# brunohs1993/Nanokappa

Measured on AMD Instinct MI355X. Metric: phonon-steps/sec (whole node), higher is better.
Workload: dtype f64

## Files before the change

### nanokappa_amd/csrc/nk_kernels.h

```cpp
#pragma once
#ifndef NK_KERNEL_LINKAGE
#define NK_KERNEL_LINKAGE
#endif
#include "nk_device.h"

#define NK_TILE 64
#ifndef NK_NT
#define NK_NT 0
#endif
#if NK_NT
#define NK_LD(p) __builtin_nontemporal_load(p)
#define NK_ST(p, v) __builtin_nontemporal_store(v, p)
#else
#define NK_LD(p) (*(p))
#define NK_ST(p, v) (*(p) = (v))
#endif
#ifdef NK_STAMPS
#define NK_STAMP(k)                                                                                    \
    do {                                                                                               \
        unsigned long long t_;                                                                         \
        __builtin_amdgcn_sched_barrier(0);                                                             \
        asm volatile("s_memtime %0\n\ts_waitcnt lgkmcnt(0)" : "=s"(t_)::"memory");                     \
        __builtin_amdgcn_sched_barrier(0);                                                             \
        st_acc[k] += t_ - st_last;                                                                     \
        st_last = t_;                                                                                  \
    } while (0)
#else
#define NK_STAMP(k) do { } while (0)
#endif

__device__ __forceinline__ int nk_rank(unsigned long long m) {
    return (int)__builtin_amdgcn_mbcnt_hi((unsigned int)(m >> 32), __builtin_amdgcn_mbcnt_lo((unsigned int)m, 0u));
}

struct NkLds {
    NkSvTab tb;
    NkBins bins;
    const double *planes, *faces;
    const NkFacet *facets;
    const double *resT;
    const int *rf_off;
    const double *rf_cdf, *rf_verts;
    unsigned int *sp_pref, *sp_cnt, *sp_rm;
    double *sp_cv, *sp_pr;
    double *lrec;
    double *carry;
    double *oring;
    unsigned int *oring_w;
    double *colsum;
};

#ifndef NK_LREC_STRIDE
#define NK_LREC_STRIDE 5
#endif
#ifndef NK_OUT_RING
#define NK_OUT_RING 0
#endif
#define NK_ORING (NK_OUT_RING ? 128 : 0)
#define NK_CARRY_DOUBLES(kind) (((kind) == 3 || (kind) == 5) ? 576 : 448)
#ifndef NK_BOX_GENERAL_CAST
#define NK_BOX_GENERAL_CAST 0
#endif
#define NK_COLSUM_DOUBLES 768
__host__ __device__ inline size_t nk_lds_bytes(int S, int R, int F, int NP, int Fc, int geom, int kind, int nrf, int rbfP, int nlrec = 0, int carry = 0) {
    const bool emit = kind == 1 || kind >= 4;
    int Fl = geom == 1 ? F : 0;
    int Pl = Fl ? NP : 0;
    int Fcl = geom == 1 ? Fc : 0;
    size_t nd = (size_t)S + (size_t)((rbfP + 1) & ~1) + 3 * S + ((3 * S) & 1) + 4 * (size_t)S + NK_NREP * S + NK_NREP * 3 * S + 4 * R +
                (size_t)Fl * NK_FACE_DOUBLES + (size_t)Pl * NK_PLANE_DOUBLES + 2 * (size_t)R + 10 * (size_t)nrf +
                (emit ? 2 * (size_t)(NK_WG / 64) * NK_EMIT_CHUNK : 0) + (kind >= 2 ? (size_t)(NK_WG / 64) * ((size_t)nlrec * 2 * NK_LREC_STRIDE + (carry ? NK_CARRY_DOUBLES(kind) : 0) + NK_ORING * ((kind == 3 || kind == 5) ? 6 : 5)) : 0) +
                (kind >= 4 ? NK_COLSUM_DOUBLES : 0) + 4;
    size_t bytes = nd * 8 + (size_t)Fcl * sizeof(NkFacet) +
                   (size_t)(NK_NREP * S + R + 1 + (R + 1) + (emit ? 3 * (NK_WG / 64) * NK_EMIT_CHUNK : 0) + (kind >= 2 ? (NK_WG / 64) * NK_ORING : 0)) * 4 + 32;
    return (bytes + 15) & ~(size_t)15;
}

template <int GEOM, int KIND>
__device__ __forceinline__ void nk_lds_carve(const NkDev &d, unsigned char *smem, NkLds &L) {
    constexpr bool EMIT = KIND == 1 || KIND >= 4;
    const int S = d.S, R = d.R;
    const int Fl = GEOM == 1 ? d.F : 0;
    const int Pl = Fl ? d.NP : 0;
    const int Fcl = GEOM == 1 ? d.Fc : 0;
    const int nrf = (GEOM == 1 && d.res_lds) ? d.res_nf : 0;
    double *p = (double *)smem;
    L.tb.Tsv = p; p += S + ((d.rbf_P + 1) & ~1);
    L.tb.cen = p; p += 3 * S + ((3 * S) & 1);
    p += ((size_t)S & 1);
    L.tb.sv = (const NkSv *)p; p += 4 * S;
    L.bins.E = p; p += NK_NREP * S;
    L.bins.flux = p; p += NK_NREP * 3 * S;
    L.bins.resb = p; p += 4 * R;
    p += ((size_t)(p - (double *)smem) & 1);
    double *faces = p; p += (size_t)Fl * NK_FACE_DOUBLES;
    double *planes = p; p += (size_t)Pl * NK_PLANE_DOUBLES;
    double *resT = p; p += 2 * R;
    double *rf_cdf = p; p += nrf;
    double *rf_verts = p; p += 9 * (size_t)nrf;
    if (EMIT) { L.sp_cv = p; p += (NK_WG / 64) * NK_EMIT_CHUNK; L.sp_pr = p; p += (NK_WG / 64) * NK_EMIT_CHUNK; } else L.sp_cv = L.sp_pr = nullptr;
    p += ((size_t)(p - (double *)smem) & 1);
    if (KIND >= 2) {
        L.lrec = p; p += (NK_WG / 64) * (size_t)d.nlrec * 2 * NK_LREC_STRIDE;
        L.carry = p; p += d.qx ? 0 : (NK_WG / 64) * NK_CARRY_DOUBLES(KIND);
        L.oring = p; p += (NK_WG / 64) * NK_ORING * ((KIND == 3 || KIND == 5) ? 6 : 5);
    } else { L.lrec = nullptr; L.carry = nullptr; L.oring = nullptr; }
    if (KIND >= 4) { L.colsum = p; p += NK_COLSUM_DOUBLES; } else L.colsum = nullptr;
    NkFacet *facets = (NkFacet *)p;
    unsigned int *u = (unsigned int *)(facets + Fcl);
    L.bins.N = u; u += NK_NREP * S;
    L.bins.nleave = u; u += R;
    L.bins.misc = u; u += 1;
    int *rf_off = (int *)u; u += R + 1;
    if (EMIT) {
        L.sp_pref = u; u += (NK_WG / 64) * NK_EMIT_CHUNK;
        L.sp_cnt = u; u += (NK_WG / 64) * NK_EMIT_CHUNK;
        L.sp_rm = u; u += (NK_WG / 64) * NK_EMIT_CHUNK;
    } else { L.sp_pref = L.sp_cnt = L.sp_rm = nullptr; }
    if (KIND >= 2) { L.oring_w = u; u += (NK_WG / 64) * NK_ORING; } else L.oring_w = nullptr;
    L.resT = resT;
    L.rf_off = rf_off; L.rf_cdf = rf_cdf; L.rf_verts = rf_verts;
    if (GEOM == 1) { L.faces = faces; L.planes = planes; L.facets = facets; }
    else { L.faces = d.faces; L.planes = d.planes; L.facets = d.facets; }
}
template <int GEOM, int KIND>
__device__ __forceinline__ void nk_lds_setup(const NkDev &d, unsigned char *smem, NkLds &L) {
    nk_lds_carve<GEOM, KIND>(d, smem, L);
    const int S = d.S, R = d.R;
    const int Fl = GEOM == 1 ? d.F : 0;
    const int Pl = Fl ? d.NP : 0;
    const int Fcl = GEOM == 1 ? d.Fc : 0;
    const int nrf = (GEOM == 1 && d.res_lds) ? d.res_nf : 0;
    double *faces = const_cast<double *>(L.faces), *planes = const_cast<double *>(L.planes);
    NkFacet *facets = const_cast<NkFacet *>(L.facets);
    double *resT = const_cast<double *>(L.resT), *rf_cdf = const_cast<double *>(L.rf_cdf), *rf_verts = const_cast<double *>(L.rf_verts);
    int *rf_off = const_cast<int *>(L.rf_off);
    double *Tsv = const_cast<double *>(L.tb.Tsv), *cen = const_cast<double *>(L.tb.cen);
    NkSv *sv = const_cast<NkSv *>(L.tb.sv);
    const int t = threadIdx.x, nth = blockDim.x;
    const int nT = S + d.rbf_P, a = d.sv_axis, nface = Fl * NK_FACE_DOUBLES, nplane = Pl * NK_PLANE_DOUBLES;
    const int nfw = Fcl * (int)(sizeof(NkFacet) / 4);
    const int jn = t + 1 < S ? t + 1 : t;
    const double l_T = t < nT ? d.T_sv[t] : 0.0;
    const double l_cen = t < 3 * S ? d.centers[t] : 0.0;
    const double l_c = t < S ? d.centers[3 * t + a] : 0.0, l_cn = t < S ? d.centers[3 * jn + a] : 0.0, l_Tn = t < S ? d.T_sv[jn] : 0.0;
    const double l_rT = t < R ? d.res_T[t] : 1.0;
    const double l_face = t < nface ? d.faces[t] : 0.0;
    const double l_plane = t < nplane ? d.planes[t] : 0.0;
    const int l_off = (nrf > 0 && t <= R) ? d.res_face_off[t] : 0;
    const double l_cdf = t < nrf ? d.res_face_cdf[t] : 0.0;
    const double l_vert = t < 9 * nrf ? d.res_face_verts[t] : 0.0;
    const int32_t l_fw = t < nfw ? ((const int32_t *)d.facets)[t] : 0;
    if (t < nT) Tsv[t] = l_T;
    if (t < 3 * S) cen[t] = l_cen;
    if (t < S) {
        NkSv q;
        q.c = l_c; q.T = l_T; q.slope = jn > t ? (l_Tn - l_T) / (l_cn - l_c) : 0.0; q.invT = 1.0 / l_T;
        sv[t] = q;
    }
    if (t < R) { L.bins.nleave[t] = 0u; resT[2 * t] = l_rT; resT[2 * t + 1] = 1.0 / l_rT; }
    if (t < nface) faces[t] = l_face;
    if (t < nplane) planes[t] = l_plane;
    if (nrf > 0 && t <= R) rf_off[t] = l_off;
    if (t < nrf) rf_cdf[t] = l_cdf;
    if (t < 9 * nrf) rf_verts[t] = l_vert;
    if (t < nfw) ((int32_t *)facets)[t] = l_fw;
    for (int i = t; i < NK_NREP * S; i += nth) { L.bins.E[i] = 0.0; L.bins.N[i] = 0u; }
    for (int i = t; i < NK_NREP * 3 * S; i += nth) L.bins.flux[i] = 0.0;
    for (int i = t; i < 4 * R; i += nth) L.bins.resb[i] = 0.0;
    if (t == 0) L.bins.misc[0] = 0u;
    for (int i = t + nth; i < nT; i += nth) Tsv[i] = d.T_sv[i];
    for (int i = t + nth; i < 3 * S; i += nth) cen[i] = d.centers[i];
    for (int i = t + nth; i < S; i += nth) {
        const int j = i + 1 < S ? i + 1 : i;
        const double c = d.centers[3 * i + a], cn = d.centers[3 * j + a], T = d.T_sv[i], Tn = d.T_sv[j];
        NkSv q;
        q.c = c; q.T = T; q.slope = j > i ? (Tn - T) / (cn - c) : 0.0; q.invT = 1.0 / T;
        sv[i] = q;
    }
    for (int i = t + nth; i < R; i += nth) { L.bins.nleave[i] = 0u; const double T = d.res_T[i]; resT[2 * i] = T; resT[2 * i + 1] = 1.0 / T; }
    for (int i = t + nth; i < nface; i += nth) faces[i] = d.faces[i];
    for (int i = t + nth; i < nplane; i += nth) planes[i] = d.planes[i];
    if (nrf > 0) {
        for (int i = t + nth; i <= R; i += nth) rf_off[i] = d.res_face_off[i];
        for (int i = t + nth; i < nrf; i += nth) rf_cdf[i] = d.res_face_cdf[i];
        for (int i = t + nth; i < 9 * nrf; i += nth) rf_verts[i] = d.res_face_verts[i];
    }
    for (int i = t + nth; i < nfw; i += nth) ((int32_t *)facets)[i] = ((const int32_t *)d.facets)[i];
    __syncthreads();
}

__device__ __forceinline__ void nk_lds_flush(const NkDev &d, const NkLds &L, int64_t row) {
    __syncthreads();
    const int S = d.S, R = d.R;
    double *out = d.partials + row * d.NB;
    for (int b = threadIdx.x; b < d.NB; b += blockDim.x) {
        double v = 0.0;
        if (b < S) { for (int r = 0; r < NK_NREP; ++r) v += L.bins.E[r * S + b]; }
        else if (b < 2 * S) { unsigned int c = 0; for (int r = 0; r < NK_NREP; ++r) c += L.bins.N[r * S + (b - S)]; v = (double)c; }
        else if (b < 5 * S) { int k = b - 2 * S; for (int r = 0; r < NK_NREP; ++r) v += L.bins.flux[r * 3 * S + k]; }
        else if (b < 5 * S + R) v = (double)L.bins.nleave[b - 5 * S];
        else if (b < 5 * S + 2 * R) v = L.bins.resb[4 * (b - 5 * S - R)];
        else if (b < 5 * S + 5 * R) { int k = b - 5 * S - 2 * R; v = L.bins.resb[4 * (k / 3) + 1 + (k % 3)]; }
        else v = (double)L.bins.misc[0];
        out[b] = v;
    }
}

struct NkSegModes {
    const NkMode *rec;
    const int32_t *gm;
    int nl;
    int estride, eoff;
    __device__ __forceinline__ int mode(int i) const { return gm ? gm[i] : i; }
    __device__ __forceinline__ int entry_mode(int l) const { return gm ? gm[l] : l * estride + eoff; }
};
struct NkPlainModes { __device__ __forceinline__ int mode(int i) const { return i; } };
__device__ __forceinline__ void nk_mode_home(const NkDev &d, int mode, int &seg, int &idx) {
    const uint32_t slot = (uint32_t)d.m2s[mode], n = (uint32_t)d.nseg;
    const uint32_t q = slot / n;
    idx = (int)q;
    seg = (int)(slot - q * n);
}
__device__ __forceinline__ NkSegModes nk_seg_modes(const NkDev &d, int seg) {
    NkSegModes sm;
    sm.rec = d.part ? d.modetab_p + (int64_t)seg * d.nlmax : d.modetab;
    sm.gm = d.part ? d.s2m + (int64_t)seg * d.nlmax : nullptr;
    sm.nl = d.seg_nl[seg];
    sm.estride = d.nseg; sm.eoff = seg;
    return sm;
}

template <bool RBF = true>
__device__ __forceinline__ double nk_relax(const NkDev &d, const NkLds &L, const NkTauWin &tw, const double4 &ra, const double4 &rb, double x,
                                           double y, double z, double occ, const NkSegModes &sm, int idx) {
    double invT;
    const double T = nk_interp_T<RBF>(d, L.tb, x, y, z, invT);
    const double tau = nk_lifetime(d, tw, rb.y, rb.z, rb.w, T, sm, idx);
    const double n0 = (T > 0.0) ? nk_be(ra.x * d.c_hk, rb.x, invT, d.invT0) : 0.0;
    const double xr = -d.dt * nk_rcp(tau);
    double er;
    if (__builtin_expect(__ballot(tau > 0.0 && !(xr > -0.125)) == 0ull, 1)) er = nk_exp_small(xr);
    else er = nk_exp(xr);
    return (tau > 0.0) ? n0 + (occ - n0) * er : n0;
}

__device__ __forceinline__ void nk_sample_res_face(const int *off, const double *cdf, const double *verts, int r, double uf,
                                                   double us, double ur, double &x0, double &y0, double &z0) {
    const int f0 = off[r], nf = off[r + 1] - f0;
    int a = nk_ss_right(cdf + f0, nf, uf);
    a = a > nf - 1 ? nf - 1 : a;
    const double *fv = verts + 9 * (f0 + a);
    const double sq = sqrt(us);
    const double a0 = 1.0 - sq, a1 = (1.0 - ur) * sq, a2 = ur * sq;
    x0 = a0 * fv[0] + a1 * fv[3] + a2 * fv[6];
    y0 = a0 * fv[1] + a1 * fv[4] + a2 * fv[7];
    z0 = a0 * fv[2] + a1 * fv[5] + a2 * fv[8];
}

#define NK_RAY(GEOM, d, L, skip, x, y, z, vx, vy, vz, tc, fc)                                                        \
    do {                                                                                                              \
        if ((GEOM) == 2 && (d).NG > 0) nk_find_boundary_tree(d, skip, x, y, z, vx, vy, vz, tc, fc);                      \
        else nk_find_boundary((L).planes, (L).faces, (d).NP, (d).tol, x, y, z, vx, vy, vz, tc, fc);                   \
    } while (0)

__device__ __forceinline__ void nk_emit_entry(const NkDev &d, uint32_t step, int64_t rm, int64_t at, double prob, int &c, int &c_mine, double &cv) {
    const double fixed = floor(prob);
    int mask;
    if (d.res_gen == 0) {
        cv = d.rc_p[(int64_t)(step & 1u) * d.rc_len + at] + (prob - fixed);
        mask = cv >= 1.0;
        cv -= (double)mask;
        d.rc_p[(int64_t)((step + 1u) & 1u) * d.rc_len + at] = cv;
    } else {
        double d1;
        nk_uniform2_dev(d.seed, (uint64_t)rm | 0xFFFFFFFF00000000ull, step, NK_TAG_DICE, cv, d1);
        mask = cv <= (prob - fixed);
    }
    c = (int)fixed + mask;
    c_mine = c;
    if (d.nranks > 1) {
        c_mine = 0;
        for (int level = c; level >= 1; --level)
            c_mine += (((uint32_t)rm + (uint32_t)level + step) % (uint32_t)d.nranks) == (uint32_t)d.rank;
    }
}

NK_KERNEL_LINKAGE __global__ __launch_bounds__(NK_WG) void k_emit_one_to_one(NkDev d, uint32_t step) {
    if (d.halt[0]) return;
    int64_t total = 0;
    for (int r = 0; r < d.R; ++r) total += d.nleave_prev[r];
    for (int64_t c = (int64_t)blockIdx.x * NK_WG + threadIdx.x; c < total; c += (int64_t)gridDim.x * NK_WG) {
        int r = 0;
        int64_t i = c;
        while (r < d.R - 1 && i >= d.nleave_prev[r]) { i -= d.nleave_prev[r]; ++r; }
        if (((uint32_t)((uint64_t)i + step) % (uint32_t)d.nranks) != (uint32_t)d.rank) continue;
        const uint64_t pid = ((uint64_t)((step + 1u) & 0xFFFFFFu) << 40) | ((uint64_t)r << 32) | (uint64_t)i;
        double um, u1;
        nk_uniform2_dev(d.seed, pid, step, NK_TAG_DICE, um, u1);
        int m = nk_ss_left(d.res_roulette + (int64_t)r * d.M, d.M, um);
        m = m > d.M - 1 ? d.M - 1 : m;
        if (i >= (1ll << 24)) { atomicOr(d.overflow, 16); continue; }
        int seg, lidx;
        if (d.part) nk_mode_home(d, m, seg, lidx); else seg = m % d.nseg;
        const int at = atomicAdd(d.sp_inbox_n + seg, 1);
        if (at < d.sp_icap) d.sp_inbox[(int64_t)seg * d.sp_icap + at] = ((uint64_t)i << 40) | ((uint64_t)((int64_t)r * d.M + m) << 12);
        else atomicOr(d.overflow, 8);
    }
}

__device__ __forceinline__ void nk_newborn_place(const NkDev &d, double x0, double y0, double z0, double vx, double vy, double vz,
                                                 double dt_in, double tc, double &x, double &y, double &z, double &nts) {
    x = x0 + vx * dt_in; y = y0 + vy * dt_in; z = z0 + vz * dt_in;
    nts = tc / d.dt - dt_in / d.dt;
}

template <int GEOM, bool BOX>
__device__ __forceinline__ int nk_emit_one(const NkDev &d, const NkLds &L, uint32_t step, int seg, int lane, unsigned int *sp_pref,
                                           unsigned int *sp_cnt, unsigned int *sp_rm, double *sp_cv, double *sp_pr, bool ahead, bool to_queue,
                                           int &bound_out
#ifdef NK_STAMPS
                                           , unsigned long long em_t0, unsigned long long em_t1, unsigned long long &em_t2
#endif
) {
    const int plo = d.seg_lo ? d.seg_lo[seg] : 0;
    const int64_t base = (int64_t)seg * d.segcap;
    const int count = d.seg_count[seg];
    const NkSegModes sm = nk_seg_modes(d, seg);
    const int nent = d.res_gen != 2 ? d.R * sm.nl : 0;
    int made = 0;
    int sp_bound = 0;
    for (int e0 = 0; e0 < nent || (d.res_gen == 2 && e0 == 0); e0 += NK_EMIT_CHUNK) {
        int spn = 0;
        if (d.res_gen == 2) {
            spn = d.sp_inbox_n[seg];
            spn = spn < d.sp_icap ? spn : d.sp_icap;
            sp_bound = lane == 0 ? 2 * spn + 64 : 0;
        } else {
            unsigned int run = 0;
#pragma unroll
            for (int k = 0; k < 2; ++k) {
                const int e = e0 + k * 64 + lane;
                int c = 0, cmine = 0;
                double cv = 0.0, prob = 0.0;
                unsigned int rm32 = 0, rl = 0;
                if (e < nent) {
                    const int r = e / sm.nl, l = e - r * sm.nl;
                    rl = ((unsigned int)r << 12) | ((unsigned int)l << 18);
                    const int64_t rm = (int64_t)r * d.M + sm.entry_mode(l);
                    const int64_t at = ((int64_t)seg * d.R + r) * d.nlmax + l;
                    prob = d.ep_p[at];
                    nk_emit_entry(d, step, rm, at, prob, c, cmine, cv);
                    rm32 = (unsigned int)rm;
                    sp_bound += ((int)floor(prob) + 1 + d.nranks - 1) / d.nranks;
                }
                unsigned int v = (unsigned int)cmine;
#pragma unroll
                for (int o = 1; o < 64; o <<= 1) { const unsigned int u = __shfl_up(v, o, 64); if (lane >= o) v += u; }
                sp_cnt[k * 64 + lane] = (unsigned int)c | rl;
                sp_rm[k * 64 + lane] = rm32;
                sp_cv[k * 64 + lane] = cv;
                sp_pr[k * 64 + lane] = prob;
                sp_pref[k * 64 + lane] = v + run - (unsigned int)cmine;
                run += __shfl(v, 63, 64);
            }
            __builtin_amdgcn_fence(__ATOMIC_SEQ_CST, "wavefront");
            spn = (int)run;
        }
#ifdef NK_STAMPS
        if (!em_t2) em_t2 = __builtin_amdgcn_s_memrealtime();
#endif
        for (int spj = 0; spj < spn; spj += NK_TILE) {
            const int j = spj + lane;
            if (j >= spn) continue;
            int64_t rm;
            int level, r, idx;
            double prob = 0.0, cval = 0.0;
            uint64_t o2o = 0;
            if (d.res_gen == 2) {
                const uint64_t recd = d.sp_inbox[(int64_t)seg * d.sp_icap + j];
                rm = (int64_t)((recd >> 12) & 0xFFFFFFFull);
                level = 0;
                o2o = recd >> 40;
                r = (int)((uint32_t)rm / (uint32_t)d.M);
                const int mode = (int)((uint32_t)rm - (uint32_t)r * (uint32_t)d.M);
                idx = d.part ? (int)((uint32_t)d.m2s[mode] / (uint32_t)d.nseg) : mode;
            } else {
                int lo = 0, hi = NK_EMIT_CHUNK;
                while (hi - lo > 1) { const int mid = (lo + hi) >> 1; if ((int)sp_pref[mid] <= j) lo = mid; else hi = mid; }
                const unsigned int cw = sp_cnt[lo];
                const int q = j - (int)sp_pref[lo], c = (int)(cw & 0xFFFu);
                r = (int)((cw >> 12) & 0x3Fu);
                rm = (int64_t)sp_rm[lo];
                idx = d.part ? (int)(cw >> 18) : (int)((uint32_t)rm - (uint32_t)r * (uint32_t)d.M);
                cval = sp_cv[lo];
                prob = sp_pr[lo];
                if (d.nranks == 1) level = c - q;
                else {
                    const uint32_t n = (uint32_t)d.nranks;
                    const uint32_t tq = ((uint32_t)d.rank + n - (((uint32_t)rm + step) % n)) % n;
                    const uint32_t top = (uint32_t)c - (((uint32_t)c + n - tq) % n);
                    level = (int)(top - (uint32_t)q * n);
                }
            }
            const NkMode *rec = sm.rec + idx;
            const double4 ra = *reinterpret_cast<const double4 *>(rec);
            const double E0 = rec->E0;
            const uint64_t pid = level > 0 ? ((uint64_t)((step + 1u) & 0xFFFFFFu) << 40) | ((uint64_t)rm << 12) | (uint64_t)level
                                           : ((uint64_t)((step + 1u) & 0xFFFFFFu) << 40) | ((uint64_t)r << 32) | o2o;
            double uf, us, ur, ut;
            nk_uniform2_dev(d.seed, pid, step, NK_TAG_EMIT, uf, us);
            nk_uniform2_dev(d.seed, pid, step, NK_TAG_EMIT + 1, ur, ut);
            const double iprob = level > 0 ? nk_rcp(prob) : 0.0;
            const double dt_in = (level == 0) ? d.dt * ut
                               : (level == 1) ? d.dt * (1.0 - cval * iprob)
                                              : d.dt * (1.0 - ((double)(level - 1) + ut) * iprob);
            double x0, y0, z0;
            if (GEOM == 1 && d.res_lds) nk_sample_res_face(L.rf_off, L.rf_cdf, L.rf_verts, r, uf, us, ur, x0, y0, z0);
            else nk_sample_res_face(d.res_face_off, d.res_face_cdf, d.res_face_verts, r, uf, us, ur, x0, y0, z0);
            const double omega = ra.x, vx = ra.y, vy = ra.z, vz = ra.w;
            const double occ = nk_be(omega * d.c_hk, E0, L.resT[2 * r + 1], d.invT0);
            if (GEOM == 2 && to_queue) {
                const int o = made + j;
                if (o < d.segcap) {
                    const int64_t i = base + o;
                    const int rf = d.res_facet[r];
                    const NkFacet &fq = d.facets[rf];
                    const int skip = nk_tree_skip(d, rf, fq.cx, fq.cy, fq.cz, fq.nx, fq.ny, fq.nz, x0, y0, z0, vx, vy, vz);
                    d.qx[i] = x0; d.qy[i] = y0; d.qz[i] = z0; d.qocc[i] = occ; d.qnts[i] = dt_in;
                    d.qw0[i] = NK_NEWBORN | ((uint32_t)((skip == rf ? rf : -1) + 1) << d.lb) | (uint32_t)idx;
                    if (d.qpid) d.qpid[i] = pid;
                } else if (!(ahead && d.halt[1])) atomicOr(d.overflow, 1);
                continue;
            }
            double tc = 0.0;
            int facet = -1;
            int skip = NK_TREE_NO_SKIP;
            if (GEOM == 2 && d.NG > 0) {
                const int rf = d.res_facet[r];
                const NkFacet &fq = d.facets[rf];
                skip = nk_tree_skip(d, rf, fq.cx, fq.cy, fq.cz, fq.nx, fq.ny, fq.nz, x0, y0, z0, vx, vy, vz);
            }
            if (!BOX) NK_RAY(GEOM, d, L, skip, x0, y0, z0, vx, vy, vz, tc, facet);
            const int o = count + made + j;
            if (plo + o < d.segcap) {
                const int64_t i = base + plo + o;
                const NkSlot q = nk_slot(d, i);
                double xa, ya, za, na;
                nk_newborn_place(d, x0, y0, z0, vx, vy, vz, dt_in, tc, xa, ya, za, na);
                d.x.p[q.od] = xa; d.y.p[q.od] = ya; d.z.p[q.od] = za;
                d.occ.p[q.od] = occ;
                if (!BOX) d.nts.p[q.od] = na;
                d.w0.p[q.ow] = BOX ? (NK_NEWBORN | (uint32_t)idx) : (NK_NEWBORN | ((uint32_t)(facet + 1) << d.lb) | (uint32_t)idx);
                if (d.pid) d.pid.p[q.od] = pid;
            } else if (!(ahead && d.halt[1])) atomicOr(d.overflow, 1);
        }
        made += spn;
        __builtin_amdgcn_fence(__ATOMIC_SEQ_CST, "wavefront");
    }
#pragma unroll
    for (int o = 32; o > 0; o >>= 1) sp_bound += __shfl_xor(sp_bound, o, 64);
    const int room = d.segcap - plo - count;
    const int put = (GEOM == 2 && to_queue) ? 0 : (made < room ? made : (room > 0 ? room : 0));
    if (lane == 0) {
        if (GEOM == 2 && to_queue) { d.seg_new[seg] = 0; d.seg_evq[seg] = made < d.segcap ? made : d.segcap; }
        else d.seg_new[seg] = put;
        d.seg_bound[seg] = sp_bound;
        if (d.res_gen == 2) d.sp_inbox_n[seg] = 0;
#ifdef NK_STAMPS
        if (d.stamps) { unsigned long long *w = d.stamps + ((int64_t)d.nseg + seg) * 8 + 4; w[0] = em_t0; w[1] = em_t1; w[2] = em_t2; w[3] = __builtin_amdgcn_s_memrealtime(); }
#endif
    }
    bound_out = sp_bound;
    return put;
}

template <int GEOM, bool BOX = false>
__device__ __forceinline__ void nk_emit_segments(const NkDev &d, NkLds L, uint32_t step, int bid, int nblocks, bool ahead
#ifdef NK_STAMPS
                                                 , unsigned long long em_t0, unsigned long long em_t1
#endif
) {
#ifdef NK_STAMPS
    unsigned long long em_t2 = 0;
#endif
    const int tid = threadIdx.x, lane = tid & 63, wave = __builtin_amdgcn_readfirstlane(tid >> 6);
    unsigned int *sp_pref = L.sp_pref + wave * NK_EMIT_CHUNK, *sp_cnt = L.sp_cnt + wave * NK_EMIT_CHUNK,
                 *sp_rm = L.sp_rm + wave * NK_EMIT_CHUNK;
    double *sp_cv = L.sp_cv + wave * NK_EMIT_CHUNK, *sp_pr = L.sp_pr + wave * NK_EMIT_CHUNK;
    const int nwaves = nblocks * (NK_WG / 64);
    const bool to_queue = GEOM == 2 && d.NG > 0 && d.qx != nullptr;
    for (int seg = bid * (NK_WG / 64) + wave; seg < d.nseg; seg += nwaves) {
        int bound_;
#ifdef NK_STAMPS
        (void)nk_emit_one<GEOM, BOX>(d, L, step, seg, lane, sp_pref, sp_cnt, sp_rm, sp_cv, sp_pr, ahead, to_queue, bound_, em_t0, em_t1, em_t2);
#else
        (void)nk_emit_one<GEOM, BOX>(d, L, step, seg, lane, sp_pref, sp_cnt, sp_rm, sp_cv, sp_pr, ahead, to_queue, bound_);
#endif
    }
}

template <int GEOM, bool BOX = false>
__device__ __forceinline__ void nk_emit_body(const NkDev &d, uint32_t step, unsigned char *smem, int bid, int nblocks, bool ahead = false) {
#ifdef NK_STAMPS
    const unsigned long long em_t0 = __builtin_amdgcn_s_memrealtime();
#endif
    if (d.halt[0]) return;
    NkLds L;
    nk_lds_setup<GEOM, 1>(d, smem, L);
#ifdef NK_STAMPS
    nk_emit_segments<GEOM, BOX>(d, L, step, bid, nblocks, ahead, em_t0, __builtin_amdgcn_s_memrealtime());
#else
    nk_emit_segments<GEOM, BOX>(d, L, step, bid, nblocks, ahead);
#endif
}

template <int GEOM, bool BOX = false>
__global__ __launch_bounds__(NK_WG) void k_emit(NkDev d, uint32_t step) {
    extern __shared__ __align__(16) unsigned char smem[];
    nk_emit_body<GEOM, BOX>(d, step, smem, (int)blockIdx.x, (int)gridDim.x);
}

template <bool PID>
struct NkOut {
    double *x, *y, *z, *occ, *nts, *pid;
    unsigned int *w0;
    int on, ob, wout;
    int64_t m0; int ms, mroom;
    __device__ __forceinline__ void place(int64_t first, int sign, int room) { m0 = first; ms = sign; mroom = room; }
    __device__ __forceinline__ void init(const NkLds &L, int wave) {
        double *p = L.oring + wave * NK_ORING * (PID ? 6 : 5);
        x = p; y = p + NK_ORING; z = p + 2 * NK_ORING; occ = p + 3 * NK_ORING; nts = p + 4 * NK_ORING; pid = PID ? p + 5 * NK_ORING : nullptr;
        w0 = L.oring_w + wave * NK_ORING;
        on = ob = wout = 0;
    }
    __device__ __forceinline__ int reserve(int rank, int n) { const int o = wout + rank; wout += n; return o; }
    template <bool BOX>
    static __device__ __forceinline__ void put_slot(const NkDev &d, int64_t i, double px, double py, double pz, double pocc, double pnts,
                                                    uint32_t pw0, unsigned long long ppid) {
        typedef NkBlock<!BOX, PID> B;
        double *q = B::slot(d.x.p, i);
        NK_ST(q, px); NK_ST(q + B::O_Y, py); NK_ST(q + B::O_Z, pz); NK_ST(q + B::O_OCC, pocc);
        if (!BOX) NK_ST(q + B::O_NTS, pnts);
        if (PID) NK_ST(reinterpret_cast<unsigned long long *>(q + B::O_PID), ppid);
        NK_ST(B::word(d.x.p, i), pw0);
    }
    template <bool BOX = false>
    __device__ __forceinline__ void store(const NkDev &d, int64_t base, bool put, int o, double px, double py, double pz, double pocc,
                                          double pnts, uint32_t pw0, unsigned long long ppid) {
        if (put) {
            if (o < mroom) put_slot<BOX>(d, m0 + ms * (int64_t)o, px, py, pz, pocc, pnts, pw0, ppid);
            else atomicOr(d.overflow, 2);
        }
    }
    template <bool BOX = false>
    __device__ __forceinline__ void push(const NkDev &d, int64_t base, int lane, bool put, int rank, int n, double px, double py,
                                         double pz, double pocc, double pnts, uint32_t pw0, unsigned long long ppid) {
        if (!NK_OUT_RING) {
            if (put) {
                const int o = wout + rank;
                if (o < mroom) put_slot<BOX>(d, m0 + ms * (int64_t)o, px, py, pz, pocc, pnts, pw0, ppid);
                else atomicOr(d.overflow, 2);
            }
            wout += n;
            return;
        }
        if (put) {
            const int e = (ob + on + rank) & (NK_ORING - 1);
            x[e] = px; y[e] = py; z[e] = pz; occ[e] = pocc; nts[e] = pnts; w0[e] = pw0;
            if (PID) pid[e] = __longlong_as_double((long long)ppid);
        }
        on += n;
        __builtin_amdgcn_fence(__ATOMIC_SEQ_CST, "wavefront");
        if (on >= NK_TILE) flush(d, base, lane, NK_TILE);
    }
    __device__ __forceinline__ void flush(const NkDev &d, int64_t base, int lane, int n) {
        if (wout + n <= d.segcap) {
            if (lane < n) {
                const int e = (ob + lane) & (NK_ORING - 1);
                const int64_t i = base + wout + lane;
                d.x[i] = x[e]; d.y[i] = y[e]; d.z[i] = z[e]; d.occ[i] = occ[e]; d.nts[i] = nts[e]; d.w0[i] = w0[e];
                if (PID) d.pid[i] = (unsigned long long)__double_as_longlong(pid[e]);
            }
            wout += n;
        } else if (lane == 0) atomicOr(d.overflow, 2);
        ob = (ob + n) & (NK_ORING - 1);
        on -= n;
        __builtin_amdgcn_fence(__ATOMIC_SEQ_CST, "wavefront");
    }
};

typedef double nk_v2d __attribute__((ext_vector_type(2)));
typedef const __attribute__((address_space(3))) nk_v2d *NkLdsRec;
__device__ __forceinline__ NkLdsRec nk_lds_rec(const double2 *q) { return (NkLdsRec)(const void *)q; }

#ifndef NK_SWEEP_OCC
#define NK_SWEEP_OCC 3
#endif
#ifndef NK_PREFETCH2
#define NK_PREFETCH2 0
#endif
#ifndef NK_PARK_TAU
#define NK_PARK_TAU 1
#endif
#ifndef NK_PRIO_ROT
#define NK_PRIO_ROT 0
#endif
#ifndef NK_DEFER_STORE
#define NK_DEFER_STORE 0
#endif
#ifndef NK_SWEEP_OCC_BIG
#define NK_SWEEP_OCC_BIG 2
#endif
#ifndef NK_SWEEP_OCC_SPLIT
#define NK_SWEEP_OCC_SPLIT 4
#endif
#define NK_SWEEP_BOUND(GEOM, ROUGH, RBF, SPLIT) ((SPLIT) ? NK_SWEEP_OCC_SPLIT : (((GEOM) == 2 || (RBF)) ? NK_SWEEP_OCC_BIG : NK_SWEEP_OCC))
template <int GEOM, bool ROUGH, bool RBF, bool PID, bool SPLIT, bool LREC, int FAST = 0, bool BOX = false>
__device__ __forceinline__ void nk_sweep_body(const NkDev &d, NkLds L, uint32_t step, int do_relax, int flags, int wg, int nwg
#ifdef NK_STAMPS
                                              , unsigned long long st_entry_r
#endif
) {
    static_assert(!BOX || (GEOM == 1 && !SPLIT && !NK_PREFETCH2 && !NK_OUT_RING), "the box store goes with the fused sweep over LDS tables");
    const bool do_flux = (flags & 1) != 0;
    const int tid = threadIdx.x, lane = tid & 63, wave = __builtin_amdgcn_readfirstlane(tid >> 6);
    const int rep = lane & (NK_NREP - 1);
    const uint32_t lbmask = (1u << d.lb) - 1u;
    NkBoxWalls bw;
    if (BOX) bw.load(d);
    NkTauWin tw;
    tw.load(d, NK_PARK_TAU != 0);
    double2 *lrec = reinterpret_cast<double2 *>(L.lrec) + wave * d.nlrec * NK_LREC_STRIDE;
    double *const cX = L.carry ? L.carry + wave * NK_CARRY_DOUBLES(PID ? 3 : 2) : nullptr;
    double *const cP = cX + 6 * 64;
    uint32_t *const cW = reinterpret_cast<uint32_t *>(cX + (PID ? 7 : 6) * 64);
    const int nwaves = nwg * (NK_WG / 64);
#if NK_PRIO_ROT
    const int prio_phase = (int)(wg / (nwg > 3 ? (nwg + 3) / 4 : 1));
#endif
    for (int seg = wg * (NK_WG / 64) + wave; seg < d.nseg; seg += nwaves) {
        const int64_t base = (int64_t)seg * d.segcap;
        const int nnew = d.R > 0 ? d.seg_new[seg] : 0;
        const int count = d.seg_count[seg] + nnew;
        if (lane == 0 && nnew > 0) atomicAdd(&L.bins.misc[0], (unsigned int)nnew);
        const NkSegModes sm = nk_seg_modes(d, seg);
        constexpr bool use_lrec = LREC;
        if (use_lrec) {
            for (int r0 = lane; r0 < sm.nl; r0 += 64) {
                const double4 *g = reinterpret_cast<const double4 *>(sm.rec + r0);
                const double4 a = g[0], b = g[1];
                double2 *q = lrec + r0 * NK_LREC_STRIDE;
                q[0] = make_double2(a.x, a.y); q[1] = make_double2(a.z, a.w); q[2] = make_double2(b.x, b.y); q[3] = make_double2(b.z, b.w);
                if (NK_LREC_STRIDE > 4 && (ROUGH || PID)) *reinterpret_cast<int *>(q + 4) = sm.mode(r0);
            }
            __builtin_amdgcn_fence(__ATOMIC_SEQ_CST, "wavefront");
        }
        auto mode_of = [&](int i) -> int {
            if (use_lrec && NK_LREC_STRIDE > 4) return *(const __attribute__((address_space(3))) int *)(const void *)(lrec + i * NK_LREC_STRIDE + 4);
            return sm.mode(i);
        };
        constexpr bool ALT = GEOM == 1 || SPLIT;
        const bool down = ALT && d.down != 0;
        const int lo = (ALT && d.seg_lo) ? d.seg_lo[seg] : 0, hi = lo + count;
        const int blo = lo & ~(NK_TILE - 1), bhi = count > 0 ? ((hi - 1) & ~(NK_TILE - 1)) : blo;
        const int nA = count > 0 ? (bhi - blo) / NK_TILE + 1 : 0;
        const int wlo = (!down && lo > (d.segcap - count) / 2) ? 0 : lo;
        NkOut<PID> O;
        O.init(L, wave);
        O.place(down ? base + hi - 1 : base + wlo, down ? -1 : 1, down ? count : d.segcap - wlo);
        int qn = SPLIT ? d.seg_evq[seg] : 0;
        if (SPLIT && lane == 0 && qn > 0) atomicAdd(&L.bins.misc[0], (unsigned int)qn);
        int cn = 0;
#ifdef NK_STAMPS
        unsigned long long st_acc[8] = {0, 0, 0, 0, 0, 0, 0, 0}, st_last;
        asm volatile("s_memtime %0\n\ts_waitcnt lgkmcnt(0)" : "=s"(st_last)::"memory");
        const unsigned long long st_c0 = st_last, st_r0 = __builtin_amdgcn_s_memrealtime();
#endif
        constexpr bool PF2 = NK_PREFETCH2 || SPLIT;
        constexpr bool DEFER = (NK_DEFER_STORE || PF2) && !NK_OUT_RING;
        struct NkTileBuf { uint32_t w0; double x, y, z, occ, nts; unsigned long long pid; };
        NkTileBuf bA = {0u, 0, 0, 0, 0, 0, 0ull}, bB = bA;
        auto fetch = [&](NkTileBuf &b, int r) {
            int rr = down ? bhi - r : blo + r;
            rr = rr < 0 ? 0 : (rr < d.segcap - NK_TILE ? rr : d.segcap - NK_TILE);
            const int64_t i0 = base + rr;
            if (PF2) {
                typedef NkBlock<!BOX, PID> B;
                const double *px = B::tile(d.x.p, i0, lane), *py = px + B::O_Y, *pz = px + B::O_Z, *po = px + B::O_OCC, *pn = px + B::O_NTS;
                const uint32_t *pw = B::word(d.x.p, i0) + lane;
                asm volatile("global_load_dword %0, %1, off" : "=v"(b.w0) : "v"(pw) : "memory");
                asm volatile("global_load_dwordx2 %0, %1, off" : "=v"(b.x) : "v"(px) : "memory");
                asm volatile("global_load_dwordx2 %0, %1, off" : "=v"(b.y) : "v"(py) : "memory");
                asm volatile("global_load_dwordx2 %0, %1, off" : "=v"(b.z) : "v"(pz) : "memory");
                asm volatile("global_load_dwordx2 %0, %1, off" : "=v"(b.occ) : "v"(po) : "memory");
                asm volatile("global_load_dwordx2 %0, %1, off" : "=v"(b.nts) : "v"(pn) : "memory");
                if (PID) { const double *pp = px + B::O_PID; asm volatile("global_load_dwordx2 %0, %1, off" : "=v"(b.pid) : "v"(pp) : "memory"); }
                return;
            }
            if (rr + lane >= lo && rr + lane < hi && r < nA * NK_TILE) {
                typedef NkBlock<!BOX, PID> B;
                const double *q = B::tile(d.x.p, i0, lane);
                b.w0 = NK_LD(B::word(d.x.p, i0) + lane); b.x = NK_LD(q); b.y = NK_LD(q + B::O_Y); b.z = NK_LD(q + B::O_Z); b.occ = NK_LD(q + B::O_OCC);
                if (!BOX) b.nts = NK_LD(q + B::O_NTS);
                if (PID) b.pid = NK_LD(reinterpret_cast<const unsigned long long *>(q + B::O_PID));
            }
        };
        auto arrived = [&](NkTileBuf &b) {
            if (!PF2) return;
            if (PID) asm volatile("s_waitcnt vmcnt(7)" : "+v"(b.w0), "+v"(b.x), "+v"(b.y), "+v"(b.z), "+v"(b.occ), "+v"(b.nts), "+v"(b.pid) : : "memory");
            else asm volatile("s_waitcnt vmcnt(6)" : "+v"(b.w0), "+v"(b.x), "+v"(b.y), "+v"(b.z), "+v"(b.occ), "+v"(b.nts) : : "memory");
        };
        auto drained = [&](NkTileBuf &b) {
            if (PF2) asm volatile("s_waitcnt vmcnt(0)" : "+v"(b.w0), "+v"(b.x), "+v"(b.y), "+v"(b.z), "+v"(b.occ), "+v"(b.nts), "+v"(b.pid) : : "memory");
        };
        fetch(bA, 0);
        if (PF2) fetch(bB, NK_TILE);
        bool sdone = false, sev = false;
        int so = 0, sq = 0;
        double sx = 0, sy = 0, sz = 0, socc = 0, snts = 0;
        uint32_t sw0 = 0u;
        unsigned long long spid = 0;
        auto turn = [&](NkTileBuf &buf, const int t) __attribute__((always_inline)) {
            const bool flush = t == nA;
            arrived(buf);
#if NK_PRIO_ROT
            if ((t & ((1 << NK_PRIO_ROT) - 1)) == 0) {
                switch (((t >> NK_PRIO_ROT) + prio_phase) & 3) {
                    case 0: __builtin_amdgcn_s_setprio(0); break;
                    case 1: __builtin_amdgcn_s_setprio(1); break;
                    case 2: __builtin_amdgcn_s_setprio(2); break;
                    default: __builtin_amdgcn_s_setprio(3); break;
                }
            }
#endif
            bool act = false;
            double x = 0, y = 0, z = 0, occ = 0, nts = 0, omega = 0, E0 = 0, vx = 0, vy = 0, vz = 0;
            uint32_t w0 = 0u;
            unsigned long long pid = 0;
            if (!flush) {
                const int r = t * NK_TILE;
                { const int rr = down ? bhi - r : blo + r; act = rr + lane >= lo && rr + lane < hi; }
                w0 = buf.w0; x = buf.x; y = buf.y; z = buf.z; occ = buf.occ; nts = buf.nts; pid = buf.pid;
            }
            if (DEFER) {
                asm volatile("" : "+v"(x), "+v"(y), "+v"(z), "+v"(occ), "+v"(nts), "+v"(w0));
                O.template store<BOX>(d, base, sdone, so, sx, sy, sz, socc, snts, sw0, spid);
                sdone = false;
                if (SPLIT && sev) {
                    if (sq < d.segcap) {
                        const int64_t i = base + sq;
                        d.qx[i] = sx; d.qy[i] = sy; d.qz[i] = sz; d.qocc[i] = socc; d.qnts[i] = snts; d.qw0[i] = sw0;
                        if (PID) d.qpid[i] = spid;
                    }
                }
                sev = false;
            }
            if (PF2) fetch(buf, (t + 2) * NK_TILE);
            if (!flush) {
                const int r = t * NK_TILE;
                if (!PF2) fetch(buf, r + NK_TILE);
                const bool newborn = (w0 & NK_NEWBORN) != 0u;
                w0 &= ~NK_NEWBORN;
                const int idx = act ? (int)(w0 & lbmask) : 0;
                double4 ra, rb;
                if (use_lrec) {
                    const NkLdsRec q = nk_lds_rec(lrec + idx * NK_LREC_STRIDE);
                    const nk_v2d q0 = q[0], q1 = q[1], q2 = q[2], q3 = q[3];
                    ra = make_double4(q0.x, q0.y, q1.x, q1.y); rb = make_double4(q2.x, q2.y, q3.x, q3.y);
                }
                else { const double4 *g = reinterpret_cast<const double4 *>(sm.rec + idx); ra = g[0]; rb = g[1]; }
                omega = ra.x; vx = ra.y; vy = ra.z; vz = ra.w; E0 = rb.x;
#ifdef NK_STAMPS
                { const double fence_ = x + omega; asm volatile("" ::"v"(fence_)); }
#endif
                NK_STAMP(0);
                if (act && !newborn) {
                    if (do_relax) occ = nk_relax<RBF>(d, L, tw, ra, rb, x, y, z, occ, sm, idx);
                    x += vx * d.dt; y += vy * d.dt; z += vz * d.dt;
                    if (!BOX) nts -= 1.0;
                }
#ifdef NK_STAMPS
                { const double fence_ = x + occ; asm volatile("" ::"v"(fence_)); }
#endif
                NK_STAMP(1);
            }
            const bool ev = BOX ? (act && (w0 & NK_LOST) == 0u && nk_box_out(bw, x, y, z, vx, vy, vz)) : (act && nts < 0.0);
            const bool done = act && !ev;
            const unsigned long long mD = __ballot(done), mE = __ballot(ev);
            if (done) nk_tally_one(d, L.tb, L.bins, x, y, z, occ, omega, E0, vx, vy, vz, do_flux, rep);
            if (DEFER) {
                so = O.reserve(nk_rank(mD), __popcll(mD));
                sdone = done; sx = x; sy = y; sz = z; socc = occ; snts = nts; sw0 = w0; spid = pid;
            } else O.template push<BOX>(d, base, lane, done, nk_rank(mD), __popcll(mD), x, y, z, occ, nts, w0, pid);
            NK_STAMP(2);
            if (SPLIT) {
                if (DEFER) { sev = ev; sq = qn + nk_rank(mE); }
                else if (ev) {
                    const int o = qn + nk_rank(mE);
                    if (o < d.segcap) {
                        const int64_t i = base + o;
                        d.qx[i] = x; d.qy[i] = y; d.qz[i] = z; d.qocc[i] = occ; d.qnts[i] = nts; d.qw0[i] = w0;
                        if (PID) d.qpid[i] = pid;
                    }
                }
                qn += __popcll(mE);
                return;
            }
            const int pn = __popcll(mE), erank = nk_rank(mE);
// ... 1628 lines not shown
```

Baseline: 53.40 billion.

## Prefetch emit segment data during LDS setup and batch per-lane mode loads

Adds a batched emit path for GEOM==1 with small reservoir counts. The first segment's header, emission probabilities, carry values and mode records are loaded into registers while the LDS setup loads are still in flight, overlapping that global latency with setup. Mode records are then shared across the wave with shuffles instead of per-entry global loads. For BOX geometry a slim setup also skips loading geometry tables into LDS. This costs more registers and adds a code path that only applies when R<=2 and nlmax<=128.

Measured after the change: 51.95 billion. 2.7% lower.

```diff
diff --git a/nanokappa_amd/csrc/nk_kernels.h b/nanokappa_amd/csrc/nk_kernels.h
--- a/nanokappa_amd/csrc/nk_kernels.h
+++ b/nanokappa_amd/csrc/nk_kernels.h
@@ -123,8 +123,8 @@
     if (GEOM == 1) { L.faces = faces; L.planes = planes; L.facets = facets; }
     else { L.faces = d.faces; L.planes = d.planes; L.facets = d.facets; }
 }
-template <int GEOM, int KIND>
-__device__ __forceinline__ void nk_lds_setup(const NkDev &d, unsigned char *smem, NkLds &L) {
+template <int GEOM, int KIND, bool SLIM, class Issued>
+__device__ __forceinline__ bool nk_lds_setup_then(const NkDev &d, unsigned char *smem, NkLds &L, Issued &&issued) {
     nk_lds_carve<GEOM, KIND>(d, smem, L);
     const int S = d.S, R = d.R;
     const int Fl = GEOM == 1 ? d.F : 0;
@@ -141,37 +141,39 @@
     const int nT = S + d.rbf_P, a = d.sv_axis, nface = Fl * NK_FACE_DOUBLES, nplane = Pl * NK_PLANE_DOUBLES;
     const int nfw = Fcl * (int)(sizeof(NkFacet) / 4);
     const int jn = t + 1 < S ? t + 1 : t;
-    const double l_T = t < nT ? d.T_sv[t] : 0.0;
-    const double l_cen = t < 3 * S ? d.centers[t] : 0.0;
-    const double l_c = t < S ? d.centers[3 * t + a] : 0.0, l_cn = t < S ? d.centers[3 * jn + a] : 0.0, l_Tn = t < S ? d.T_sv[jn] : 0.0;
+    const double l_T = (!SLIM && t < nT) ? d.T_sv[t] : 0.0;
+    const double l_cen = (!SLIM && t < 3 * S) ? d.centers[t] : 0.0;
+    const bool svt = !SLIM && t < S;
+    const double l_c = svt ? d.centers[3 * t + a] : 0.0, l_cn = svt ? d.centers[3 * jn + a] : 0.0, l_Tn = svt ? d.T_sv[jn] : 0.0;
     const double l_rT = t < R ? d.res_T[t] : 1.0;
-    const double l_face = t < nface ? d.faces[t] : 0.0;
-    const double l_plane = t < nplane ? d.planes[t] : 0.0;
+    const double l_face = (!SLIM && t < nface) ? d.faces[t] : 0.0;
+    const double l_plane = (!SLIM && t < nplane) ? d.planes[t] : 0.0;
     const int l_off = (nrf > 0 && t <= R) ? d.res_face_off[t] : 0;
     const double l_cdf = t < nrf ? d.res_face_cdf[t] : 0.0;
     const double l_vert = t < 9 * nrf ? d.res_face_verts[t] : 0.0;
-    const int32_t l_fw = t < nfw ? ((const int32_t *)d.facets)[t] : 0;
-    if (t < nT) Tsv[t] = l_T;
-    if (t < 3 * S) cen[t] = l_cen;
-    if (t < S) {
+    const int32_t l_fw = (!SLIM && t < nfw) ? ((const int32_t *)d.facets)[t] : 0;
+    if (issued()) return false;
+    if (!SLIM && t < nT) Tsv[t] = l_T;
+    if (!SLIM && t < 3 * S) cen[t] = l_cen;
+    if (svt) {
         NkSv q;
         q.c = l_c; q.T = l_T; q.slope = jn > t ? (l_Tn - l_T) / (l_cn - l_c) : 0.0; q.invT = 1.0 / l_T;
         sv[t] = q;
     }
     if (t < R) { L.bins.nleave[t] = 0u; resT[2 * t] = l_rT; resT[2 * t + 1] = 1.0 / l_rT; }
-    if (t < nface) faces[t] = l_face;
-    if (t < nplane) planes[t] = l_plane;
+    if (!SLIM && t < nface) faces[t] = l_face;
+    if (!SLIM && t < nplane) planes[t] = l_plane;
     if (nrf > 0 && t <= R) rf_off[t] = l_off;
     if (t < nrf) rf_cdf[t] = l_cdf;
     if (t < 9 * nrf) rf_verts[t] = l_vert;
-    if (t < nfw) ((int32_t *)facets)[t] = l_fw;
+    if (!SLIM && t < nfw) ((int32_t *)facets)[t] = l_fw;
     for (int i = t; i < NK_NREP * S; i += nth) { L.bins.E[i] = 0.0; L.bins.N[i] = 0u; }
     for (int i = t; i < NK_NREP * 3 * S; i += nth) L.bins.flux[i] = 0.0;
     for (int i = t; i < 4 * R; i += nth) L.bins.resb[i] = 0.0;
     if (t == 0) L.bins.misc[0] = 0u;
-    for (int i = t + nth; i < nT; i += nth) Tsv[i] = d.T_sv[i];
-    for (int i = t + nth; i < 3 * S; i += nth) cen[i] = d.centers[i];
-    for (int i = t + nth; i < S; i += nth) {
+    for (int i = t + nth; !SLIM && i < nT; i += nth) Tsv[i] = d.T_sv[i];
+    for (int i = t + nth; !SLIM && i < 3 * S; i += nth) cen[i] = d.centers[i];
+    for (int i = t + nth; !SLIM && i < S; i += nth) {
         const int j = i + 1 < S ? i + 1 : i;
         const double c = d.centers[3 * i + a], cn = d.centers[3 * j + a], T = d.T_sv[i], Tn = d.T_sv[j];
         NkSv q;
@@ -179,15 +181,20 @@
         sv[i] = q;
     }
     for (int i = t + nth; i < R; i += nth) { L.bins.nleave[i] = 0u; const double T = d.res_T[i]; resT[2 * i] = T; resT[2 * i + 1] = 1.0 / T; }
-    for (int i = t + nth; i < nface; i += nth) faces[i] = d.faces[i];
-    for (int i = t + nth; i < nplane; i += nth) planes[i] = d.planes[i];
+    for (int i = t + nth; !SLIM && i < nface; i += nth) faces[i] = d.faces[i];
+    for (int i = t + nth; !SLIM && i < nplane; i += nth) planes[i] = d.planes[i];
     if (nrf > 0) {
         for (int i = t + nth; i <= R; i += nth) rf_off[i] = d.res_face_off[i];
         for (int i = t + nth; i < nrf; i += nth) rf_cdf[i] = d.res_face_cdf[i];
         for (int i = t + nth; i < 9 * nrf; i += nth) rf_verts[i] = d.res_face_verts[i];
     }
-    for (int i = t + nth; i < nfw; i += nth) ((int32_t *)facets)[i] = ((const int32_t *)d.facets)[i];
+    for (int i = t + nth; !SLIM && i < nfw; i += nth) ((int32_t *)facets)[i] = ((const int32_t *)d.facets)[i];
     __syncthreads();
+    return true;
+}
+template <int GEOM, int KIND>
+__device__ __forceinline__ void nk_lds_setup(const NkDev &d, unsigned char *smem, NkLds &L) {
+    (void)nk_lds_setup_then<GEOM, KIND, false>(d, smem, L, [] { return false; });
 }
 
 __device__ __forceinline__ void nk_lds_flush(const NkDev &d, const NkLds &L, int64_t row) {
@@ -264,11 +271,13 @@
         else nk_find_boundary((L).planes, (L).faces, (d).NP, (d).tol, x, y, z, vx, vy, vz, tc, fc);                   \
     } while (0)
 
-__device__ __forceinline__ void nk_emit_entry(const NkDev &d, uint32_t step, int64_t rm, int64_t at, double prob, int &c, int &c_mine, double &cv) {
+template <bool PRE = false>
+__device__ __forceinline__ void nk_emit_entry(const NkDev &d, uint32_t step, int64_t rm, int64_t at, double prob, int &c, int &c_mine, double &cv,
+                                              double rc_pre = 0.0) {
     const double fixed = floor(prob);
     int mask;
     if (d.res_gen == 0) {
-        cv = d.rc_p[(int64_t)(step & 1u) * d.rc_len + at] + (prob - fixed);
+        cv = (PRE ? rc_pre : d.rc_p[(int64_t)(step & 1u) * d.rc_len + at]) + (prob - fixed);
         mask = cv >= 1.0;
         cv -= (double)mask;
         d.rc_p[(int64_t)((step + 1u) & 1u) * d.rc_len + at] = cv;
@@ -315,24 +324,77 @@
     nts = tc / d.dt - dt_in / d.dt;
 }
 
-template <int GEOM, bool BOX>
+struct NkEmitBatch {
+    int hdr;
+    __device__ __forceinline__ int plo() const { return __builtin_amdgcn_readlane(hdr, 0); }
+    __device__ __forceinline__ int count() const { return __builtin_amdgcn_readlane(hdr, 1); }
+    __device__ __forceinline__ int nl() const { return __builtin_amdgcn_readlane(hdr, 2); }
+    double ep[2][2], rc[2][2];
+    int gm[2];
+    double4 ra[2];
+    double E0[2];
+};
+__device__ __forceinline__ bool nk_emit_batched(const NkDev &d) {
+    return d.part && d.res_gen != 2 && d.R <= 2 && d.nlmax <= 2 * 64 && d.ep_p != nullptr && d.modetab_p != nullptr;
+}
+__device__ __forceinline__ void nk_emit_fetch(const NkDev &d, uint32_t step, int seg, int lane, NkEmitBatch &b) {
+    const int32_t *lo = d.seg_lo ? d.seg_lo : d.seg_count;
+    const int h0 = lane == 0 ? lo[seg] : 0, h1 = lane == 1 ? d.seg_count[seg] : 0, h2 = lane == 2 ? d.seg_nl[seg] : 0;
+    b.hdr = h0 | h1 | h2;
+    const double *rc = d.rc_p + (int64_t)(step & 1u) * d.rc_len;
+#pragma unroll
+    for (int h = 0; h < 2; ++h) {
+        const int l = lane + 64 * h;
+        const bool ok = l < d.nlmax;
+        const int64_t sl = (int64_t)seg * d.nlmax + l;
+        b.gm[h] = ok ? d.s2m[sl] : 0;
+#pragma unroll
+        for (int r = 0; r < 2; ++r) {
+            const int64_t at = ((int64_t)seg * d.R + r) * d.nlmax + l;
+            b.ep[r][h] = (ok && r < d.R) ? d.ep_p[at] : 0.0;
+            b.rc[r][h] = (ok && r < d.R && d.res_gen == 0) ? rc[at] : 0.0;
+        }
+    }
+#pragma unroll
+    for (int h = 0; h < 2; ++h) {
+        const int l = lane + 64 * h;
+        const NkMode *rec = d.modetab_p + (int64_t)seg * d.nlmax + l;
+        if (l < d.nlmax) { b.ra[h] = *reinterpret_cast<const double4 *>(rec); b.E0[h] = rec->E0; }
+        else { b.ra[h] = make_double4(0.0, 0.0, 0.0, 0.0); b.E0[h] = 0.0; }
+    }
+}
+
+template <int GEOM, bool BOX, bool PRE = false>
 __device__ __forceinline__ int nk_emit_one(const NkDev &d, const NkLds &L, uint32_t step, int seg, int lane, unsigned int *sp_pref,
                                            unsigned int *sp_cnt, unsigned int *sp_rm, double *sp_cv, double *sp_pr, bool ahead, bool to_queue,
-                                           int &bound_out
+                                           int &bound_out, const NkEmitBatch &pb
 #ifdef NK_STAMPS
                                            , unsigned long long em_t0, unsigned long long em_t1, unsigned long long &em_t2
 #endif
 ) {
-    const int plo = d.seg_lo ? d.seg_lo[seg] : 0;
+    const int plo = PRE ? (d.seg_lo ? pb.plo() : 0) : (d.seg_lo ? d.seg_lo[seg] : 0);
     const int64_t base = (int64_t)seg * d.segcap;
-    const int count = d.seg_count[seg];
-    const NkSegModes sm = nk_seg_modes(d, seg);
+    const int count = PRE ? pb.count() : d.seg_count[seg];
+    NkSegModes sm;
+    if (PRE) { sm.rec = nullptr; sm.gm = nullptr; sm.nl = pb.nl(); sm.estride = d.nseg; sm.eoff = seg; }
+    else sm = nk_seg_modes(d, seg);
     const int nent = d.res_gen != 2 ? d.R * sm.nl : 0;
     int made = 0;
     int sp_bound = 0;
     for (int e0 = 0; e0 < nent || (d.res_gen == 2 && e0 == 0); e0 += NK_EMIT_CHUNK) {
         int spn = 0;
-        if (d.res_gen == 2) {
+        if (PRE) {
+#pragma unroll
+            for (int h = 0; h < 2; ++h) {
+#pragma unroll
+                for (int r = 0; r < 2; ++r) {
+                    const int l = lane + 64 * h, e = r * sm.nl + l - e0;
+                    if (l < sm.nl && r < d.R && e >= 0 && e < NK_EMIT_CHUNK) { sp_pr[e] = pb.ep[r][h]; sp_cv[e] = pb.rc[r][h]; sp_rm[e] = (unsigned int)pb.gm[h]; }
+                }
+            }
+            __builtin_amdgcn_fence(__ATOMIC_SEQ_CST, "wavefront");
+        }
+        if (!PRE && d.res_gen == 2) {
             spn = d.sp_inbox_n[seg];
             spn = spn < d.sp_icap ? spn : d.sp_icap;
             sp_bound = lane == 0 ? 2 * spn + 64 : 0;
@@ -347,10 +409,10 @@
                 if (e < nent) {
                     const int r = e / sm.nl, l = e - r * sm.nl;
                     rl = ((unsigned int)r << 12) | ((unsigned int)l << 18);
-                    const int64_t rm = (int64_t)r * d.M + sm.entry_mode(l);
+                    const int64_t rm = (int64_t)r * d.M + (PRE ? (int)sp_rm[k * 64 + lane] : sm.entry_mode(l));
                     const int64_t at = ((int64_t)seg * d.R + r) * d.nlmax + l;
-                    prob = d.ep_p[at];
-                    nk_emit_entry(d, step, rm, at, prob, c, cmine, cv);
+                    prob = PRE ? sp_pr[k * 64 + lane] : d.ep_p[at];
+                    nk_emit_entry<PRE>(d, step, rm, at, prob, c, cmine, cv, PRE ? sp_cv[k * 64 + lane] : 0.0);
                     rm32 = (unsigned int)rm;
                     sp_bound += ((int)floor(prob) + 1 + d.nranks - 1) / d.nranks;
                 }
@@ -372,12 +434,12 @@
 #endif
         for (int spj = 0; spj < spn; spj += NK_TILE) {
             const int j = spj + lane;
-            if (j >= spn) continue;
+            if (!PRE && j >= spn) continue;
             int64_t rm;
             int level, r, idx;
             double prob = 0.0, cval = 0.0;
             uint64_t o2o = 0;
-            if (d.res_gen == 2) {
+            if (!PRE && d.res_gen == 2) {
                 const uint64_t recd = d.sp_inbox[(int64_t)seg * d.sp_icap + j];
                 rm = (int64_t)((recd >> 12) & 0xFFFFFFFull);
                 level = 0;
@@ -403,9 +465,23 @@
                     level = (int)(top - (uint32_t)q * n);
                 }
             }
-            const NkMode *rec = sm.rec + idx;
-            const double4 ra = *reinterpret_cast<const double4 *>(rec);
-            const double E0 = rec->E0;
+            double4 ra;
+            double E0;
+            if (PRE) {
+                const int src = idx & 63;
+                ra.x = __shfl(pb.ra[0].x, src, 64); ra.y = __shfl(pb.ra[0].y, src, 64); ra.z = __shfl(pb.ra[0].z, src, 64);
+                ra.w = __shfl(pb.ra[0].w, src, 64); E0 = __shfl(pb.E0[0], src, 64);
+                if (d.nlmax > 64) {
+                    const double hx = __shfl(pb.ra[1].x, src, 64), hy = __shfl(pb.ra[1].y, src, 64), hz = __shfl(pb.ra[1].z, src, 64);
+                    const double hw = __shfl(pb.ra[1].w, src, 64), hE = __shfl(pb.E0[1], src, 64);
+                    if (idx >= 64) { ra.x = hx; ra.y = hy; ra.z = hz; ra.w = hw; E0 = hE; }
+                }
+                if (j >= spn) continue;
+            } else {
+                const NkMode *rec = sm.rec + idx;
+                ra = *reinterpret_cast<const double4 *>(rec);
+                E0 = rec->E0;
+            }
             const uint64_t pid = level > 0 ? ((uint64_t)((step + 1u) & 0xFFFFFFu) << 40) | ((uint64_t)rm << 12) | (uint64_t)level
                                            : ((uint64_t)((step + 1u) & 0xFFFFFFu) << 40) | ((uint64_t)r << 32) | o2o;
             double uf, us, ur, ut;
@@ -490,12 +566,48 @@
     double *sp_cv = L.sp_cv + wave * NK_EMIT_CHUNK, *sp_pr = L.sp_pr + wave * NK_EMIT_CHUNK;
     const int nwaves = nblocks * (NK_WG / 64);
     const bool to_queue = GEOM == 2 && d.NG > 0 && d.qx != nullptr;
+    const NkEmitBatch none{};
     for (int seg = bid * (NK_WG / 64) + wave; seg < d.nseg; seg += nwaves) {
         int bound_;
 #ifdef NK_STAMPS
-        (void)nk_emit_one<GEOM, BOX>(d, L, step, seg, lane, sp_pref, sp_cnt, sp_rm, sp_cv, sp_pr, ahead, to_queue, bound_, em_t0, em_t1, em_t2);
+        (void)nk_emit_one<GEOM, BOX>(d, L, step, seg, lane, sp_pref, sp_cnt, sp_rm, sp_cv, sp_pr, ahead, to_queue, bound_, none, em_t0, em_t1, em_t2);
 #else
-        (void)nk_emit_one<GEOM, BOX>(d, L, step, seg, lane, sp_pref, sp_cnt, sp_rm, sp_cv, sp_pr, ahead, to_queue, bound_);
+        (void)nk_emit_one<GEOM, BOX>(d, L, step, seg, lane, sp_pref, sp_cnt, sp_rm, sp_cv, sp_pr, ahead, to_queue, bound_, none);
+#endif
+    }
+}
+
+template <bool BOX>
+__device__ __forceinline__ void nk_emit_body_batched(const NkDev &d, uint32_t step, unsigned char *smem, int bid, int nblocks, bool ahead
+#ifdef NK_STAMPS
+                                                     , unsigned long long em_t0
+#endif
+) {
+    const int tid = threadIdx.x, lane = tid & 63, wave = __builtin_amdgcn_readfirstlane(tid >> 6);
+    const int nwaves = nblocks * (NK_WG / 64);
+    int seg = bid * (NK_WG / 64) + wave;
+    NkEmitBatch pb{};
+    NkLds L;
+    const bool go = nk_lds_setup_then<1, 1, BOX>(d, smem, L, [&] {
+        const int halted = d.halt[0];
+        if (seg < d.nseg) nk_emit_fetch(d, step, seg, lane, pb);
+        return halted != 0;
+    });
+    if (!go) return;
+#ifdef NK_STAMPS
+    const unsigned long long em_t1 = __builtin_amdgcn_s_memrealtime();
+    unsigned long long em_t2 = 0;
+#endif
+    unsigned int *sp_pref = L.sp_pref + wave * NK_EMIT_CHUNK, *sp_cnt = L.sp_cnt + wave * NK_EMIT_CHUNK,
+                 *sp_rm = L.sp_rm + wave * NK_EMIT_CHUNK;
+    double *sp_cv = L.sp_cv + wave * NK_EMIT_CHUNK, *sp_pr = L.sp_pr + wave * NK_EMIT_CHUNK;
+    for (bool first = true; seg < d.nseg; seg += nwaves, first = false) {
+        if (!first) nk_emit_fetch(d, step, seg, lane, pb);
+        int bound_;
+#ifdef NK_STAMPS
+        (void)nk_emit_one<1, BOX, true>(d, L, step, seg, lane, sp_pref, sp_cnt, sp_rm, sp_cv, sp_pr, ahead, false, bound_, pb, em_t0, em_t1, em_t2);
+#else
+        (void)nk_emit_one<1, BOX, true>(d, L, step, seg, lane, sp_pref, sp_cnt, sp_rm, sp_cv, sp_pr, ahead, false, bound_, pb);
 #endif
     }
 }
@@ -505,6 +617,16 @@
 #ifdef NK_STAMPS
     const unsigned long long em_t0 = __builtin_amdgcn_s_memrealtime();
 #endif
+    if constexpr (GEOM == 1) {
+        if (nk_emit_batched(d)) {
+#ifdef NK_STAMPS
+            nk_emit_body_batched<BOX>(d, step, smem, bid, nblocks, ahead, em_t0);
+#else
+            nk_emit_body_batched<BOX>(d, step, smem, bid, nblocks, ahead);
+#endif
+            return;
+        }
+    }
     if (d.halt[0]) return;
     NkLds L;
     nk_lds_setup<GEOM, 1>(d, smem, L);
```
